# csiro-icvg/Diff3DHPE

Measured on NVIDIA B200. Metric: denoised_pose_frames_per_s, higher is better.
Workload: dtype fp16 main + block-scaled e2m1 (mxfp4) correction products (1.5 tensor-pipe units), fp32 accumulate

## Files before the change

diff3dhpe_b200/csrc/attention_tc.cu:

```cuda
#include <cstdlib>
#include "kernels.cuh"
#include "operand.cuh"
#define D3D_MBAR_SUSPEND_NS 0
#include "ptx.cuh"

namespace d3d {
namespace {

constexpr int kTcThreads = 384;
constexpr int kCtrlRegs = 40, kSoftmaxRegs = 216;
static_assert(2 * 128 * (kSoftmaxRegs - 168) <= 128 * (168 - kCtrlRegs), "setmaxnreg pool overdrawn");
constexpr int kSpatialRows = 7 * 17;
constexpr int kTile = 128 * 128;
constexpr int kSlotCols = 256;
constexpr int kOCol = 128;
constexpr float kScaleLog2e = 0.125f * 1.4426950408889634f;

constexpr int kMaxStages = 4;
template <int NSLOT>
struct TcBars {
  uint64_t full[kMaxStages];
  uint64_t stage_free[kMaxStages];
  uint64_t s_full[NSLOT];
  uint64_t p_full[NSLOT];
  uint64_t o_full[NSLOT];
  uint64_t tmem_free[NSLOT];
  uint64_t vlo_full[NSLOT];
  uint64_t staged[NSLOT];
  uint64_t stg_free[NSLOT];
  uint32_t tmem_base;
};

#ifndef D3D_ATTN_STORE_WARP
#define D3D_ATTN_STORE_WARP 1
#endif

__device__ __forceinline__ float ex2_approx(float x) {
  float y;
  asm("ex2.approx.ftz.f32 %0, %1;" : "=f"(y) : "f"(x));
  return y;
}
__device__ __forceinline__ float rcp_approx(float x) {
  float y;
  asm("rcp.approx.ftz.f32 %0, %1;" : "=f"(y) : "f"(x));
  return y;
}
__device__ __forceinline__ uint32_t pack_f16x2(float lo, float hi) {
  uint32_t r;
  asm("cvt.rn.f16x2.f32 %0, %1, %2;" : "=r"(r) : "f"(hi), "f"(lo));
  return r;
}
__device__ __forceinline__ uint64_t make_desc_mn_sw128(uint32_t smem_addr) {
  uint64_t d = 0;
  d |= static_cast<uint64_t>((smem_addr & 0x3ffffu) >> 4);
  d |= static_cast<uint64_t>(1) << 16;
  d |= static_cast<uint64_t>(1024 >> 4) << 32;
  d |= static_cast<uint64_t>(1) << 46;
  d |= static_cast<uint64_t>(2) << 61;
  return d;
}


__device__ __forceinline__ float row_sum(const ptx::f32x2 (&ls)[2]) {
  float a, b, c, d;
  ptx::unpack2(ls[0], a, b);
  ptx::unpack2(ls[1], c, d);
  return (a + b) + (c + d);
}

template <int NCH>
__device__ __forceinline__ float softmax_row(uint32_t taddr, int F, int n_chunks_rt) {
  constexpr int kMax = NCH > 0 ? NCH : 8;
  const int n = NCH > 0 ? NCH : n_chunks_rt;
  uint32_t a0[32], a1[32], b0[32], b1[32];
  float mx[4] = {-INFINITY, -INFINITY, -INFINITY, -INFINITY};
  auto full = [&](int c) { return (NCH > 0 && c < NCH - 1) || (c + 1) * 32 <= F; };
  auto max_chunk = [&](const uint32_t (&rr)[32], int c) {
    if (full(c)) {
#pragma unroll
      for (int e = 0; e < 32; ++e) mx[e & 3] = fmaxf(mx[e & 3], __uint_as_float(rr[e]));
    } else {
#pragma unroll
      for (int e = 0; e < 32; ++e)
        if (c * 32 + e < F) mx[e & 3] = fmaxf(mx[e & 3], __uint_as_float(rr[e]));
    }
  };
  ptx::tmem_ld_32x32(taddr, a0);
  if (1 < n) ptx::tmem_ld_32x32(taddr + 32, a1);
#pragma unroll
  for (int c = 0; c < kMax; c += 4) {
    if (c < n) {
      ptx::tmem_ld_wait();
      if (c + 2 < n) ptx::tmem_ld_32x32(taddr + (c + 2) * 32, b0);
      if (c + 3 < n) ptx::tmem_ld_32x32(taddr + (c + 3) * 32, b1);
      max_chunk(a0, c);
      if (c + 1 < n) max_chunk(a1, c + 1);
    }
    if (c + 2 < n) {
      ptx::tmem_ld_wait();
      if (c + 4 < n) ptx::tmem_ld_32x32(taddr + (c + 4) * 32, a0);
      if (c + 5 < n) ptx::tmem_ld_32x32(taddr + (c + 5) * 32, a1);
      max_chunk(b0, c + 2);
      if (c + 3 < n) max_chunk(b1, c + 3);
    }
  }
  ptx::tmem_ld_32x32(taddr, a0);
  if (1 < n) ptx::tmem_ld_32x32(taddr + 32, a1);
  const float nmxs = -fmaxf(fmaxf(mx[0], mx[1]), fmaxf(mx[2], mx[3])) * kScaleLog2e;
  ptx::f32x2 ls[2] = {ptx::splat2(0.f), ptx::splat2(0.f)};
  const ptx::f32x2 sc2 = ptx::splat2(kScaleLog2e), nm2 = ptx::splat2(nmxs);
  auto exp_chunk = [&](const uint32_t (&rr)[32], int c) {
    uint32_t pk[16];
    const bool whole = full(c);
#pragma unroll
    for (int e = 0; e < 16; ++e) {
      float t0, t1;
      ptx::unpack2(ptx::fma2(ptx::pack2(__uint_as_float(rr[2 * e]), __uint_as_float(rr[2 * e + 1])), sc2, nm2), t0, t1);
      const int col = c * 32 + 2 * e;
      const float e0 = (whole || col < F) ? ex2_approx(t0) : 0.f;
      const float e1 = (whole || col + 1 < F) ? ex2_approx(t1) : 0.f;
      ls[e & 1] = ptx::add2(ls[e & 1], ptx::pack2(e0, e1));
      pk[e] = pack_f16x2(e0, e1);
    }
    ptx::tmem_st_32x16(taddr + c * 16, pk);
  };
#pragma unroll
  for (int c = 0; c < kMax; c += 4) {
    if (c < n) {
      ptx::tmem_ld_wait();
      if (c + 2 < n) ptx::tmem_ld_32x32(taddr + (c + 2) * 32, b0);
      if (c + 3 < n) ptx::tmem_ld_32x32(taddr + (c + 3) * 32, b1);
      exp_chunk(a0, c);
      if (c + 1 < n) exp_chunk(a1, c + 1);
    }
    if (c + 2 < n) {
      ptx::tmem_ld_wait();
      if (c + 4 < n) ptx::tmem_ld_32x32(taddr + (c + 4) * 32, a0);
      if (c + 5 < n) ptx::tmem_ld_32x32(taddr + (c + 5) * 32, a1);
      exp_chunk(b0, c + 2);
      if (c + 3 < n) exp_chunk(b1, c + 3);
    }
  }
  ptx::tmem_st_wait();
  return rcp_approx(row_sum(ls));
}

template <int CS, int FR>
__device__ __forceinline__ float spatial_window(const uint32_t (&a)[32], const uint32_t (&b)[32], const uint32_t (&c)[32],
                                                uint32_t (&pk0)[16], uint32_t (&pk1)[16], uint32_t (&pk2)[16]) {
  constexpr int L = 17 * FR - 32 * CS;
  static_assert(L >= 0 && L + 17 <= 96, "frame window outside the loaded chunks");
  float sv[18];
#pragma unroll
  for (int k = 0; k < 17; ++k) {
    const int li = L + k;
    sv[k] = __uint_as_float(li < 32 ? a[li & 31] : li < 64 ? b[li & 31] : c[li & 31]);
  }
  sv[17] = sv[16];
  float mx = sv[0];
#pragma unroll
  for (int k = 1; k < 17; k += 2) mx = fmaxf(mx, fmaxf(sv[k], sv[k + 1]));
  const ptx::f32x2 sc2 = ptx::splat2(kScaleLog2e), nm2 = ptx::splat2(-mx * kScaleLog2e);
  float ev[18];
  ptx::f32x2 ls = ptx::splat2(0.f);
#pragma unroll
  for (int k = 0; k < 18; k += 2) {
    float t0, t1;
    ptx::unpack2(ptx::fma2(ptx::pack2(sv[k], sv[k + 1]), sc2, nm2), t0, t1);
    ev[k] = ex2_approx(t0);
    ev[k + 1] = k + 1 < 17 ? ex2_approx(t1) : 0.f;
    ls = ptx::add2(ls, ptx::pack2(ev[k], ev[k + 1]));
  }
#pragma unroll
  for (int pi = L / 2; pi <= (L + 16) / 2; ++pi) {
    const int k0 = 2 * pi - L, k1 = k0 + 1;
    const uint32_t v = pack_f16x2(k0 >= 0 && k0 < 17 ? ev[k0 < 0 ? 0 : k0] : 0.f, k1 >= 0 && k1 < 17 ? ev[k1] : 0.f);
    if (pi < 16) pk0[pi & 15] = v;
    else if (pi < 32) pk1[pi & 15] = v;
    else pk2[pi & 15] = v;
  }
  float s0, s1;
  ptx::unpack2(ls, s0, s1);
  return s0 + s1;
}

__device__ __forceinline__ float softmax_row_spatial(uint32_t taddr, int row_l, int wq) {
  const int cs = wq >> 1;
  uint32_t a[32], b[32], c[32];
  ptx::tmem_ld_32x32(taddr + cs * 32, a);
  ptx::tmem_ld_32x32(taddr + cs * 32 + 32, b);
  ptx::tmem_ld_32x32(taddr + cs * 32 + 64, c);
  uint32_t pk0[16], pk1[16], pk2[16], z[16];
#pragma unroll
  for (int e = 0; e < 16; ++e) pk0[e] = pk1[e] = pk2[e] = z[e] = 0u;
// ... 6 lines not shown
      case 1: sum = spatial_window<0, 1>(a, b, c, pk0, pk1, pk2); break;
      case 2: sum = spatial_window<0, 2>(a, b, c, pk0, pk1, pk2); break;
      default: sum = spatial_window<0, 3>(a, b, c, pk0, pk1, pk2); break;
    }
  } else {
    switch (fr) {
      case 3: sum = spatial_window<1, 3>(a, b, c, pk0, pk1, pk2); break;
      case 4: sum = spatial_window<1, 4>(a, b, c, pk0, pk1, pk2); break;
      case 5: sum = spatial_window<1, 5>(a, b, c, pk0, pk1, pk2); break;
      default: sum = spatial_window<1, 6>(a, b, c, pk0, pk1, pk2); break;
    }
  }
  __syncwarp();
  ptx::tmem_st_32x16(taddr + cs * 16, pk0);
  ptx::tmem_st_32x16(taddr + cs * 16 + 16, pk1);
  ptx::tmem_st_32x16(taddr + cs * 16 + 32, pk2);
  ptx::tmem_st_32x16(taddr + (cs == 0 ? 48 : 0), z);
  ptx::tmem_st_wait();
  return rcp_approx(sum);
}

__device__ __forceinline__ float softmax_row_packed(uint32_t taddr, int F, int G, int row_l) {
  const int jj = row_l & (G - 1);
  const uint32_t vm = (G == 4 ? 0x11111111u : 0x55555555u) << jj;
  const int nk = F * G;
  uint32_t sv[4][32];
#pragma unroll
  for (int c = 0; c < 4; ++c) ptx::tmem_ld_32x32(taddr + c * 32, sv[c]);
  ptx::tmem_ld_wait();
  float mx = -INFINITY;
#pragma unroll
  for (int c = 0; c < 4; ++c)
#pragma unroll
    for (int e = 0; e < 32; ++e)
      if (((vm >> e) & 1u) && c * 32 + e < nk) mx = fmaxf(mx, __uint_as_float(sv[c][e]));
  const ptx::f32x2 sc2 = ptx::splat2(kScaleLog2e), nm2 = ptx::splat2(-mx * kScaleLog2e);
  ptx::f32x2 ls = ptx::splat2(0.f);
#pragma unroll
  for (int c = 0; c < 4; ++c) {
    uint32_t pk[16];
#pragma unroll
    for (int e = 0; e < 16; ++e) {
      float t0, t1;
      ptx::unpack2(ptx::fma2(ptx::pack2(__uint_as_float(sv[c][2 * e]), __uint_as_float(sv[c][2 * e + 1])), sc2, nm2), t0, t1);
      const int col = c * 32 + 2 * e;
      const float e0 = (((vm >> (2 * e)) & 1u) && col < nk) ? ex2_approx(t0) : 0.f;
      const float e1 = (((vm >> (2 * e + 1)) & 1u) && col + 1 < nk) ? ex2_approx(t1) : 0.f;
      ls = ptx::add2(ls, ptx::pack2(e0, e1));
      pk[e] = pack_f16x2(e0, e1);
    }
    ptx::tmem_st_32x16(taddr + c * 16, pk);
  }
  ptx::tmem_st_wait();
  float s0, s1;
  ptx::unpack2(ls, s0, s1);
  return rcp_approx(s0 + s1);
}

template <int FMT, int NSLOT, int NCH, bool SPATIAL, bool PACKED = false>
__global__ void __launch_bounds__((4 * NSLOT + 4) * 32, 1)
attn_temporal_tc_kernel(const __grid_constant__ CUtensorMap tm_qkv, const __grid_constant__ CUtensorMap tm_hi,
                        const __grid_constant__ CUtensorMap tm_second, const __grid_constant__ CUtensorMap tm_hi_tail,
                        const __grid_constant__ CUtensorMap tm_second_tail, uint8_t* __restrict__ sf_out, int F, int J,
                        int n_units, int n_mt, int NKp, int n_stage, int pk_g = 1, int j_tok = 0) {
  static_assert(!PACKED || (!SPATIAL && NCH == 0), "the packed mode is a temporal mode with a runtime chunk count");
  static_assert(NSLOT == 2 || (NSLOT == 3 && FMT == FMT_F4C && (SPATIAL || PACKED)), "three slots: single-tile F4C modes only");
  constexpr int kSC = NSLOT == 2 ? kSlotCols : 128;
  constexpr int kOC = NSLOT == 2 ? kOCol : 64;
  constexpr int kStgSlot = NSLOT == 2 ? kTile : 8192;
  constexpr int kTmemCols = NSLOT == 2 ? 512 : 512;
  constexpr int kSmxRegs = NSLOT == 2 ? kSoftmaxRegs : 152;
  static_assert(NSLOT != 3 || 3 * 128 * (152 - 128) <= 128 * (128 - kCtrlRegs), "setmaxnreg pool overdrawn");
  extern __shared__ __align__(1024) uint8_t smem_raw[];
  uint8_t* smem = reinterpret_cast<uint8_t*>((reinterpret_cast<uintptr_t>(smem_raw) + 1023) & ~uintptr_t(1023));
  const int stage_bytes = 3 * n_mt * kTile;
  uint8_t* StgAll = smem + n_stage * stage_bytes;
  TcBars<NSLOT>* bars = reinterpret_cast<TcBars<NSLOT>*>(StgAll + NSLOT * kStgSlot);

  const int warp = threadIdx.x >> 5, lane = threadIdx.x & 31;
  constexpr int kTmaWarp = 4 * NSLOT, kMmaWarp = 4 * NSLOT + 1;
  const int n_local = blockIdx.x < n_units ? (n_units - 1 - static_cast<int>(blockIdx.x)) / static_cast<int>(gridDim.x) + 1 : 0;
  const int W = n_local * n_mt;

  if (warp == kTmaWarp && ptx::elect_one()) {
    ptx::prefetch_tensormap(&tm_qkv);
    ptx::prefetch_tensormap(&tm_hi);
    ptx::prefetch_tensormap(&tm_second);
    for (int s = 0; s < n_stage; ++s) {
      ptx::mbar_init(&bars->full[s], 1);
      ptx::mbar_init(&bars->stage_free[s], n_mt);
    }
#pragma unroll
    for (int s = 0; s < NSLOT; ++s) {
      ptx::mbar_init(&bars->s_full[s], 1);
      ptx::mbar_init(&bars->p_full[s], 128);
      ptx::mbar_init(&bars->o_full[s], 1);
      ptx::mbar_init(&bars->tmem_free[s], 128);
      ptx::mbar_init(&bars->vlo_full[s], 1);
// ... 103 lines not shown
      ptx::bulk_wait_all();
    }
  } else {
    asm volatile("setmaxnreg.inc.sync.aligned.u32 %0;" ::"n"(kSmxRegs));
    const int slot = warp >> 2;
    const int row_l = (warp & 3) * 32 + lane;
    const uint32_t taddr = tmem_base + slot * kSC + (static_cast<uint32_t>((warp & 3) * 32) << 16);
    const int n_chunks = (NKp + 31) >> 5;
    if (!SPATIAL && NCH > 0 && (n_chunks != NCH || F <= 32 * (NCH - 1))) __trap();
    if ((SPATIAL || PACKED) && (n_mt != 1 || NKp != 128)) __trap();
    const int sw = (row_l & 7) << 4;
    const bool issuer = row_l == 0;
    uint8_t* Stg = StgAll + slot * kStgSlot;
    for (int w = slot; w < W; w += NSLOT) {
      const int n = w / n_mt, m = w - n * n_mt;
      const int i = w / NSLOT, stage = n % n_stage;
      const int unit = blockIdx.x + n * gridDim.x;
      const int seq = unit >> 3, h = unit & 7;
      int b = seq / J, j = seq - b * J;
      const bool tail = SPATIAL && j == J - 1 && F % 7 != 0;
      if (SPATIAL) { j = (b * F + 7 * j) * 17; b = 0; }
      if (PACKED) j *= pk_g;
      uint8_t* Qs = smem + stage * stage_bytes;
      const uint8_t* Vs = Qs + 2 * n_mt * kTile;
      const int r = m * 128 + row_l;
      ptx::mbar_wait(&bars->s_full[slot], i & 1);
      ptx::tc_fence_after();
      if (issuer) {
        ptx::mbar_arrive_expect_tx(&bars->vlo_full[slot], kTile);
        ptx::tma_load_4d(Qs + m * kTile, &tm_qkv, &bars->vlo_full[slot], 3 * kC + h * kHd, j, m * 128, b);
      }
      const float inv = SPATIAL ? softmax_row_spatial(taddr, row_l, warp & 3)
                      : PACKED  ? softmax_row_packed(taddr, F, pk_g, row_l)
                                : softmax_row<NCH>(taddr, F, n_chunks);
      ptx::tc_fence_before();
      ptx::mbar_arrive(&bars->p_full[slot]);

      ptx::mbar_wait(&bars->vlo_full[slot], i & 1);
      uint8_t* hi_row = Qs + m * kTile + row_l * 128;
      const uint8_t* v_row = Vs + static_cast<size_t>(r) * 128;
      ptx::f32x2 nv[32];
      {
        uint4 vh[8], vl[8];
#pragma unroll
        for (int g = 0; g < 8; ++g) {
          vh[g] = *reinterpret_cast<const uint4*>(v_row + ((g << 4) ^ sw));
          vl[g] = *reinterpret_cast<const uint4*>(hi_row + ((g << 4) ^ sw));
        }
#pragma unroll
        for (int g = 0; g < 8; ++g) {
          const uint32_t vhw[4] = {vh[g].x, vh[g].y, vh[g].z, vh[g].w};
          const uint32_t vlw[4] = {vl[g].x, vl[g].y, vl[g].z, vl[g].w};
#pragma unroll
          for (int e = 0; e < 4; ++e) {
            const float2 a = __half22float2(*reinterpret_cast<const __half2*>(&vhw[e]));
            const float2 c = __half22float2(*reinterpret_cast<const __half2*>(&vlw[e]));
            float s0, s1;
            ptx::unpack2(ptx::add2(ptx::pack2(a.x, a.y), ptx::pack2(c.x, c.y)), s0, s1);
            nv[4 * g + e] = ptx::pack2(-s0, -s1);
          }
        }
      }

      ptx::mbar_wait(&bars->o_full[slot], i & 1);
      ptx::tc_fence_after();
      uint32_t o0[32], o1[32];
      ptx::tmem_ld_32x32(taddr + kOC, o0);
      ptx::tmem_ld_32x32(taddr + kOC + 32, o1);
      ptx::tmem_ld_wait();
      ptx::tc_fence_before();
      ptx::mbar_arrive(&bars->tmem_free[slot]);

      if (D3D_ATTN_STORE_WARP) {
        if (i > 0) ptx::mbar_wait(&bars->stg_free[slot], (i - 1) & 1);
      } else {
        ptx::bar_sync(1 + slot, 128);
      }
      const ptx::f32x2 inv2 = ptx::splat2(inv);
      if (FMT == FMT_F4C) {
        float ax[2] = {0.f, 0.f}, al[2] = {0.f, 0.f};
#pragma unroll
        for (int g = 0; g < 8; ++g) {
          uint32_t hw[4];
#pragma unroll
          for (int e = 0; e < 4; ++e) {
            uint32_t& ra = g < 4 ? o0[8 * g + 2 * e] : o1[8 * (g & 3) + 2 * e];
            uint32_t& rb = g < 4 ? o0[8 * g + 2 * e + 1] : o1[8 * (g & 3) + 2 * e + 1];
            float x0, x1;
            ptx::unpack2(ptx::fma2(ptx::pack2(__uint_as_float(ra), __uint_as_float(rb)), inv2, nv[4 * g + e]), x0, x1);
            const __half2 h01 = __floats2half2_rn(x0, x1);
            const float2 hf = __half22float2(h01);
            hw[e] = *reinterpret_cast<const uint32_t*>(&h01);
            ax[g >> 2] = fmaxf(ax[g >> 2], fmaxf(fabsf(x0), fabsf(x1)));
            al[g >> 2] = fmaxf(al[g >> 2], fmaxf(fabsf(x0 - hf.x), fabsf(x1 - hf.y)));
            ra = __float_as_uint(x0);
            rb = __float_as_uint(x1);
          }
          *reinterpret_cast<uint4*>(hi_row + ((g << 4) ^ sw)) = make_uint4(hw[0], hw[1], hw[2], hw[3]);
        }
        const uint32_t bp0 = op_ue8m0_of(ax[0]), bp1 = op_ue8m0_of(ax[1]), bq0 = op_ue8m0_of(al[0]), bq1 = op_ue8m0_of(al[1]);
        uint32_t pw[8], qw[8];
#pragma unroll
        for (int g = 0; g < 8; ++g) {
          const ptx::f32x2 ip = ptx::splat2(op_ue8m0_inv(g < 4 ? bp0 : bp1)), iq = ptx::splat2(op_ue8m0_inv(g < 4 ? bq0 : bq1));
          uint32_t pa = 0, qa = 0;
#pragma unroll
          for (int e = 0; e < 4; ++e) {
            const float x0 = __uint_as_float(g < 4 ? o0[8 * g + 2 * e] : o1[8 * (g & 3) + 2 * e]);
            const float x1 = __uint_as_float(g < 4 ? o0[8 * g + 2 * e + 1] : o1[8 * (g & 3) + 2 * e + 1]);
            const float2 hf = __half22float2(__floats2half2_rn(x0, x1));
            float a0, a1, l0, l1;
            ptx::unpack2(ptx::mul2(ptx::pack2(x0, x1), ip), a0, a1);
            ptx::unpack2(ptx::mul2(ptx::sub2(ptx::pack2(x0, x1), ptx::pack2(hf.x, hf.y)), iq), l0, l1);
            pa |= op_e2m1x2(a0, a1) << (8 * e);
            qa |= op_e2m1x2(l0, l1) << (8 * e);
          }
          pw[g] = pa; qw[g] = qa;
        }
        {
          uint4* stp = reinterpret_cast<uint4*>(Stg + row_l * 32);
          stp[0] = make_uint4(pw[0], pw[1], pw[2], pw[3]);
          stp[1] = make_uint4(pw[4], pw[5], pw[6], pw[7]);
          stp[256] = make_uint4(qw[0], qw[1], qw[2], qw[3]);
          stp[257] = make_uint4(qw[4], qw[5], qw[6], qw[7]);
        }
        const int pf = PACKED ? row_l / pk_g : 0, pj = PACKED ? j + (row_l & (pk_g - 1)) : 0;
        const int64_t tok = SPATIAL  ? static_cast<int64_t>(j) + row_l
// ... 462 lines not shown
}

int make_attn_tc_maps_spatial(AttnTcMaps* maps, const __half* qkv, __half* o_hi, __half* o_second, int fmt,
                              int64_t tokens, int F) {
  const int tail_rows = (F % 7) ? (F % 7) * 17 : kSpatialRows;
  if (encode_tokens_2d(&maps->o_hi_tail, o_hi, CU_TENSOR_MAP_DATA_TYPE_FLOAT16, 2, kC, tokens, tail_rows,
                       CU_TENSOR_MAP_SWIZZLE_128B))
    return -1;
  if (fmt == FMT_F8C   ? encode_tokens_2d(&maps->o_second_tail, o_second, CU_TENSOR_MAP_DATA_TYPE_UINT8, 1, 2 * kC, tokens,
                                          tail_rows, CU_TENSOR_MAP_SWIZZLE_NONE)
      : fmt == FMT_F4C ? encode_tokens_2d(&maps->o_second_tail, o_second, CU_TENSOR_MAP_DATA_TYPE_UINT8, 1, kC, tokens,
                                          tail_rows, CU_TENSOR_MAP_SWIZZLE_NONE, 32)
                       : encode_tokens_2d(&maps->o_second_tail, o_second, CU_TENSOR_MAP_DATA_TYPE_FLOAT16, 2, kC, tokens,
                                          tail_rows, CU_TENSOR_MAP_SWIZZLE_128B))
    return -1;
  if (encode_tokens_2d(&maps->qkv, const_cast<__half*>(qkv), CU_TENSOR_MAP_DATA_TYPE_FLOAT16, 2, kQkvRow, tokens, 128,
                       CU_TENSOR_MAP_SWIZZLE_128B))
    return -1;
  if (encode_tokens_2d(&maps->o_hi, o_hi, CU_TENSOR_MAP_DATA_TYPE_FLOAT16, 2, kC, tokens, kSpatialRows,
                       CU_TENSOR_MAP_SWIZZLE_128B))
    return -1;
  if (fmt == FMT_F8C)
    return encode_tokens_2d(&maps->o_second, o_second, CU_TENSOR_MAP_DATA_TYPE_UINT8, 1, 2 * kC, tokens, kSpatialRows,
                            CU_TENSOR_MAP_SWIZZLE_NONE);
  if (fmt == FMT_F4C)
    return encode_tokens_2d(&maps->o_second, o_second, CU_TENSOR_MAP_DATA_TYPE_UINT8, 1, kC, tokens, kSpatialRows,
                            CU_TENSOR_MAP_SWIZZLE_NONE, 32);
  return encode_tokens_2d(&maps->o_second, o_second, CU_TENSOR_MAP_DATA_TYPE_FLOAT16, 2, kC, tokens, kSpatialRows,
                          CU_TENSOR_MAP_SWIZZLE_128B);
}

cudaError_t configure_attention_tc() {
  cudaError_t e;
#define D3D_CFG_TC(FMT_, NCH_, SP_)                                                                                       \
  if ((e = cudaFuncSetAttribute(attn_temporal_tc_kernel<FMT_, 2, NCH_, SP_>, cudaFuncAttributeMaxDynamicSharedMemorySize, \
                                tc_smem_bytes<2>(2))) != cudaSuccess)                                                    \
    return e;
  D3D_CFG_TC(FMT_SPLIT16, 0, false) D3D_CFG_TC(FMT_F8C, 0, false) D3D_CFG_TC(FMT_SPLIT16, 3, false)
  D3D_CFG_TC(FMT_F8C, 3, false) D3D_CFG_TC(FMT_SPLIT16, 8, false) D3D_CFG_TC(FMT_F8C, 8, false)
  D3D_CFG_TC(FMT_SPLIT16, 0, true) D3D_CFG_TC(FMT_F8C, 0, true)
  D3D_CFG_TC(FMT_F4C, 0, false) D3D_CFG_TC(FMT_F4C, 3, false) D3D_CFG_TC(FMT_F4C, 8, false) D3D_CFG_TC(FMT_F4C, 0, true)
#undef D3D_CFG_TC
  if ((e = cudaFuncSetAttribute(attn_temporal_tc_kernel<FMT_F4C, 3, 0, true>, cudaFuncAttributeMaxDynamicSharedMemorySize,
                                tc_smem_bytes<3>(1))) != cudaSuccess)
    return e;
  if ((e = cudaFuncSetAttribute(attn_temporal_tc_kernel<FMT_F4C, 3, 0, false, true>, cudaFuncAttributeMaxDynamicSharedMemorySize,
                                tc_smem_bytes<3>(1))) != cudaSuccess)
    return e;
  for (auto kern : {attn_temporal_tc2_kernel<8>, attn_temporal_tc2_kernel<3>, attn_temporal_tc2_kernel<0>})
    if ((e = cudaFuncSetAttribute(kern, cudaFuncAttributeMaxDynamicSharedMemorySize, tc_smem_bytes<2>(2))) != cudaSuccess) return e;
#define D3D_CFG_PK(FMT_)                                                                                                     \
  if ((e = cudaFuncSetAttribute(attn_temporal_tc_kernel<FMT_, 2, 0, false, true>, cudaFuncAttributeMaxDynamicSharedMemorySize, \
                                tc_smem_bytes<2>(1))) != cudaSuccess)                                                        \
    return e;
  D3D_CFG_PK(FMT_SPLIT16) D3D_CFG_PK(FMT_F8C) D3D_CFG_PK(FMT_F4C)
#undef D3D_CFG_PK
  return cudaSuccess;
}

cudaError_t launch_attn_temporal_tc(const AttnTcMaps& maps, const __half* qkv, uint8_t* o_sf, int fmt, int B, int F, int J,
                                    int num_sms, cudaStream_t st, int wg2) {
  if (B <= 0) return cudaSuccess;
  if (F < 1 || F > 256) return cudaErrorInvalidValue;
  if (fmt == FMT_F4C && !o_sf) return cudaErrorInvalidValue;
  if (F <= 64) {
    const int G = packed_group(F), JG = (J + G - 1) / G;
    const int64_t units64 = static_cast<int64_t>(B) * JG * kHeads;
    if (units64 > 0x7fffffff) return cudaErrorInvalidValue;
    const int n_units = static_cast<int>(units64);
    const int grid = n_units < num_sms ? n_units : num_sms;
    const int smem = tc_smem_bytes<2>(1);
#define D3D_LAUNCH_PK(FMT_)                                                                   \
  attn_temporal_tc_kernel<FMT_, 2, 0, false, true><<<grid, kTcThreads, smem, st>>>(           \
      maps.qkv, maps.o_hi, maps.o_second, maps.o_hi, maps.o_second, o_sf, F, JG, n_units, 1, 128, tc_stages(1), G, J)
    if (fmt == FMT_F4C && three_slots())
      attn_temporal_tc_kernel<FMT_F4C, 3, 0, false, true><<<grid, 512, tc_smem_bytes<3>(1), st>>>(
          maps.qkv, maps.o_hi, maps.o_second, maps.o_hi, maps.o_second, o_sf, F, JG, n_units, 1, 128, tc_stages(1), G, J);
    else if (fmt == FMT_F4C) D3D_LAUNCH_PK(FMT_F4C);
    else if (fmt == FMT_F8C) D3D_LAUNCH_PK(FMT_F8C);
    else D3D_LAUNCH_PK(FMT_SPLIT16);
#undef D3D_LAUNCH_PK
    return cudaGetLastError();
  }
  const int n_mt = (F + 127) / 128;
  const int NKp = (F + 15) / 16 * 16;
  const int n_units = B * J * kHeads;
  const int n_chunks = (NKp + 31) / 32;
  const int nch = (n_chunks == 8 && F > 224) ? 8 : ((n_chunks == 3 && F > 64) ? 3 : 0);
  const int grid = n_units < num_sms ? n_units : num_sms;
  const int smem = tc_smem_bytes<2>(n_mt);
#define D3D_LAUNCH_TC(FMT_, NCH_)                                                                               \
  attn_temporal_tc_kernel<FMT_, 2, NCH_, false><<<grid, kTcThreads, smem, st>>>(                      \
      maps.qkv, maps.o_hi, maps.o_second, maps.o_hi, maps.o_second, o_sf, F, J, n_units, n_mt, NKp, tc_stages(n_mt))
  if (fmt == FMT_F4C && wg2) {
    if (!o_sf) return cudaErrorInvalidValue;
#define D3D_LAUNCH_TC2(NCH_)                                                       \
  attn_temporal_tc2_kernel<NCH_><<<grid, kTc2Threads, smem, st>>>(maps.qkv, maps.o_hi, maps.o_second, o_sf, F, J, n_units, \
                                                                   n_mt, NKp, tc_stages(n_mt))
    if (nch == 8) D3D_LAUNCH_TC2(8); else if (nch == 3) D3D_LAUNCH_TC2(3); else D3D_LAUNCH_TC2(0);
#undef D3D_LAUNCH_TC2
  } else if (fmt == FMT_F4C) {
    if (!o_sf) return cudaErrorInvalidValue;
    if (nch == 8) D3D_LAUNCH_TC(FMT_F4C, 8); else if (nch == 3) D3D_LAUNCH_TC(FMT_F4C, 3); else D3D_LAUNCH_TC(FMT_F4C, 0);
  } else if (fmt == FMT_F8C) {
    if (nch == 8) D3D_LAUNCH_TC(FMT_F8C, 8); else if (nch == 3) D3D_LAUNCH_TC(FMT_F8C, 3); else D3D_LAUNCH_TC(FMT_F8C, 0);
  } else {
    if (nch == 8) D3D_LAUNCH_TC(FMT_SPLIT16, 8); else if (nch == 3) D3D_LAUNCH_TC(FMT_SPLIT16, 3); else D3D_LAUNCH_TC(FMT_SPLIT16, 0);
  }
#undef D3D_LAUNCH_TC
  return cudaGetLastError();
}

cudaError_t launch_attn_spatial_tc(const AttnTcMaps& maps, uint8_t* o_sf, int fmt, int B, int F, int num_sms,
                                   cudaStream_t st) {
  if (B <= 0) return cudaSuccess;
  const int G = (F + 6) / 7;
  const int64_t units64 = static_cast<int64_t>(B) * G * kHeads;
  if (units64 > 0x7fffffff) return cudaErrorInvalidValue;
  const int n_units = static_cast<int>(units64);
  const int grid = n_units < num_sms ? n_units : num_sms;
  const int smem = tc_smem_bytes<2>(1);
  if (fmt == FMT_F4C && three_slots()) {
    if (!o_sf) return cudaErrorInvalidValue;
    attn_temporal_tc_kernel<FMT_F4C, 3, 0, true><<<grid, 512, tc_smem_bytes<3>(1), st>>>(
        maps.qkv, maps.o_hi, maps.o_second, maps.o_hi_tail, maps.o_second_tail, o_sf, F, G, n_units, 1, 128, tc_stages(1));
  } else if (fmt == FMT_F4C) {
    if (!o_sf) return cudaErrorInvalidValue;
    attn_temporal_tc_kernel<FMT_F4C, 2, 0, true><<<grid, kTcThreads, smem, st>>>(
        maps.qkv, maps.o_hi, maps.o_second, maps.o_hi_tail, maps.o_second_tail, o_sf, F, G, n_units, 1, 128, tc_stages(1));
  } else if (fmt == FMT_F8C) {
    attn_temporal_tc_kernel<FMT_F8C, 2, 0, true><<<grid, kTcThreads, smem, st>>>(
        maps.qkv, maps.o_hi, maps.o_second, maps.o_hi_tail, maps.o_second_tail, o_sf, F, G, n_units, 1, 128, tc_stages(1));
  } else {
    attn_temporal_tc_kernel<FMT_SPLIT16, 2, 0, true><<<grid, kTcThreads, smem, st>>>(
        maps.qkv, maps.o_hi, maps.o_second, maps.o_hi_tail, maps.o_second_tail, o_sf, F, G, n_units, 1, 128, tc_stages(1));
  }
  return cudaGetLastError();
}

}
```

diff3dhpe_b200/csrc/engine.cu:

```cuda
#include <cuda_fp16.h>
#include <cuda_runtime.h>

#include <algorithm>
#include <cmath>
#include <cstdio>
#include <cstdlib>
#include <cstring>
#include <map>
#include <string>
#include <vector>

#include "../../include/diff3d_b200.h"
#include "kernels.cuh"
#include "operand.cuh"

using namespace d3d;

namespace {

std::string g_create_error;

struct Lin {
  int N = 0, K = 0;
  __half* hi = nullptr;
// ... 294 lines not shown

int run_attention(d3d_handle* h, const __half* qkv, __half* o_hi, __half* o_lo, float* o_f32, int B, bool spatial,
                  int mode, cudaStream_t st) {
  const int64_t T_all = static_cast<int64_t>(B) * h->F * h->J;
  const bool tc_path = mode == D3D_ATTN_DEFAULT && qkv == h->QKV &&
                       (spatial ? (h->have_attn_sp && h->J == 17 && env_int("D3D_ATTN_TC_SPATIAL", 1))
                                : (h->have_attn_tc && env_int("D3D_ATTN_TC", 1)));
  if (h->fmt == FMT_F4C && !o_f32 && !(tc_path && attn_tc_has_f4c())) {
    if (o_hi != h->ATT.hi || o_lo != h->ATT.lo) return fail(h, -2, "attention output must be the ATT operand");
    float* scratch = reinterpret_cast<float*>(h->H.hi);
    int r = run_attention(h, qkv, nullptr, nullptr, scratch, B, spatial, mode == D3D_ATTN_DEFAULT ? D3D_ATTN_MMA_SYNC : mode, st);
    if (r) return r;
    KLP(spatial ? D3D_PROF_ATTN_SPATIAL : D3D_PROF_ATTN_TEMPORAL, st,
        launch_split(scratch, h->ATT.hi, h->ATT.lo, h->ATT.sf, T_all, kC, FMT_F4C, 0, st));
    return 0;
  }
  if (spatial) {
    if (mode == D3D_ATTN_SIMT || h->J != 17) {
      KLP(D3D_PROF_ATTN_SPATIAL, st, launch_attn_generic_simt(qkv, o_hi, o_lo, o_f32, h->fmt, B * h->F, h->J, h->J, 1, 1, st));
    } else if (tc_path && (h->fmt != FMT_F4C || attn_tc_has_f4c())) {
      if (!o_f32 && (o_hi != h->ATT.hi || o_lo != h->ATT.lo)) return fail(h, -2, "attention output must be the ATT operand");
      const int64_t T = static_cast<int64_t>(B) * h->F * h->J;
      KLP(D3D_PROF_ATTN_SPATIAL, st, launch_attn_spatial_tc(h->attn_sp, h->ATT.sf, h->fmt, B, h->F, h->num_sms, st));
      if (o_f32) KL(launch_merge(h->ATT.hi, h->ATT.lo, h->ATT.sf, o_f32, T, kC, h->fmt, st));
    } else {
      KLP(D3D_PROF_ATTN_SPATIAL, st, launch_attn_spatial(qkv, o_hi, o_lo, o_f32, h->fmt, static_cast<int64_t>(B) * h->F, h->J, st));
    }
  } else {
    if (mode == D3D_ATTN_SIMT) {
      KLP(D3D_PROF_ATTN_TEMPORAL, st, launch_attn_temporal_simt(qkv, o_hi, o_lo, o_f32, h->fmt, B, h->F, h->J, st));
    } else if (tc_path && (h->fmt != FMT_F4C || attn_tc_has_f4c())) {
      if (!o_f32 && (o_hi != h->ATT.hi || o_lo != h->ATT.lo)) return fail(h, -2, "attention output must be the ATT operand");
      KLP(D3D_PROF_ATTN_TEMPORAL, st, launch_attn_temporal_tc(h->attn_tc, qkv, h->ATT.sf, h->fmt, B, h->F, h->J, h->num_sms, st,
                                                              env_int("D3D_ATTN_WG2", 0)));
      if (o_f32) KL(launch_merge(h->ATT.hi, h->ATT.lo, h->ATT.sf, o_f32, static_cast<int64_t>(B) * h->F * h->J, kC, h->fmt, st));
    } else {
      KLP(D3D_PROF_ATTN_TEMPORAL, st, launch_attn_temporal_mma(qkv, o_hi, o_lo, o_f32, h->fmt, B, h->F, h->J, st));
    }
  }
  return 0;
}

int check_weights(d3d_handle* h) {
  static const char* per_blk[] = {"norm1.weight", "norm1.bias", "attn.qkv.weight", "attn.proj.weight", "attn.proj.bias",
                                  "norm2.weight", "norm2.bias", "mlp.fc1.weight", "mlp.fc1.bias", "mlp.fc2.weight",
                                  "mlp.fc2.bias"};
  std::vector<std::string> need = {"fusion_layer.weight", "fusion_layer.bias", "Spatial_pos_embed", "Temporal_pos_embed",
                                   "Spatial_norm.weight", "Spatial_norm.bias", "Temporal_norm.weight", "Temporal_norm.bias",
                                   "head.0.weight", "head.0.bias", "head.1.weight", "head.1.bias"};
  if (h->cfg.with_time_emb) {
    need.insert(need.end(), {"time_mlp.1.weight", "time_mlp.1.bias", "time_mlp.3.weight", "time_mlp.3.bias"});
  }
  for (int i = 0; i < h->cfg.depth; ++i)
    for (const char* kind : {"STEblocks.", "TTEblocks."}) {
      for (const char* s : per_blk) need.push_back(std::string(kind) + std::to_string(i) + "." + s);
      if (h->cfg.with_time_emb) {
        need.push_back(std::string(kind) + std::to_string(i) + ".time_mlp.1.weight");
        need.push_back(std::string(kind) + std::to_string(i) + ".time_mlp.1.bias");
      }
    }
  for (auto& n : need)
    if (!h->loaded.count(n)) return fail(h, -30, "weights not loaded: missing tensor '" + n + "'");
  for (auto& b : h->blk)
    if (b.fold_dirty) return fail(h, -30, "internal: norm2 / fc1 of a block were not folded");
  return 0;
}

// ... 908 lines not shown
```

diff3dhpe_b200/csrc/kernels.cuh:

```cuda
#pragma once
#include <cuda.h>
#include <cuda_fp16.h>
#include <cuda_runtime.h>
#include <stdint.h>

namespace d3d {

constexpr int kC = 512;
constexpr int kHeads = 8;
constexpr int kHd = 64;
constexpr int kHidden = 1024;

enum GemmEpi { EPI_F32 = 0, EPI_GELU_SPLIT = 1, EPI_QKV16 = 2, EPI_F32_LN = 3, EPI_F32_EMIT = 4, EPI_GELU_DLN = 5,
               EPI_F32_RED = 6 };

constexpr int kQkvRow = 4 * kC;

struct GemmParams {
  int M, N, K;
  const float* bias;
  const float* residual;
  float* out_f32;
  __half* out_hi;
  __half* out_lo;
// ... 67 lines not shown
cudaError_t launch_head_ddim(const float* X, LnParams post, LnParams head_ln, const float* wh ,
                             const float* bh, DdimStep s, float* y, const float* noise, float* out3,
                             float* trace_y, float* trace_x0, int trace_stride, int trace_idx, int64_t T,
                             cudaStream_t st);

cudaError_t launch_tta_merge(const float* y, const float* yf, const int32_t* perm , float scale,
                             float* out, int64_t n_frames, int J, cudaStream_t st);
cudaError_t launch_mpjpe(const float* pred, const float* gt, const uint8_t* mask, int64_t n_frames, int J,
                         double* acc, cudaStream_t st);

cudaError_t launch_pose_metrics(const float* pred, const float* gt, const int64_t* sel , int64_t n_sel, int J,
                                double* acc, double* vel_tmp, cudaStream_t st);

cudaError_t launch_window_gather(const float* seq2d, const int64_t* start, const int32_t* perm , float* x2d,
                                 float* x2d_flip , int64_t n_win, int F, int J, cudaStream_t st);
cudaError_t launch_window_scatter(const float* pred, const int64_t* start, const int32_t* first_valid, float* seq3d,
                                  int64_t n_win, int F, int J, cudaStream_t st);

cudaError_t launch_attn_spatial(const __half* qkv, __half* o_hi, __half* o_lo, float* o_f32, int fmt, int64_t n_groups,
                                int J, cudaStream_t st);
cudaError_t launch_attn_temporal_mma(const __half* qkv, __half* o_hi, __half* o_lo, float* o_f32, int fmt, int B, int F,
                                     int J, cudaStream_t st);
struct AttnTcMaps {
  CUtensorMap qkv, o_hi, o_second;
  CUtensorMap o_hi_tail, o_second_tail;
};
int make_attn_tc_maps(AttnTcMaps* maps, const __half* qkv, __half* o_hi, __half* o_second, int fmt, int F, int J,
                      int64_t max_clips);
int make_attn_tc_maps_spatial(AttnTcMaps* maps, const __half* qkv, __half* o_hi, __half* o_second, int fmt, int64_t tokens,
                              int F);
cudaError_t launch_attn_spatial_tc(const AttnTcMaps& maps, uint8_t* o_sf, int fmt, int B, int F, int num_sms, cudaStream_t st);
cudaError_t configure_attention_tc();
cudaError_t launch_attn_temporal_tc(const AttnTcMaps& maps, const __half* qkv, uint8_t* o_sf, int fmt, int B, int F, int J,
                                    int num_sms, cudaStream_t st, int wg2 = 0);
cudaError_t launch_attn_temporal_simt(const __half* qkv, __half* o_hi, __half* o_lo, float* o_f32, int fmt, int B, int F,
                                      int J, cudaStream_t st);
cudaError_t launch_attn_generic_simt(const __half* qkv, __half* o_hi, __half* o_lo, float* o_f32, int fmt, int n_seq,
                                     int N, int64_t seq_stride_tokens_outer, int inner, int64_t tok_stride,
                                     cudaStream_t st);
cudaError_t launch_pack_qkv16(const float* qkv_f32, __half* out, int64_t T, cudaStream_t st);

cudaError_t launch_t_to_f32(const int64_t* t, int R, float* out, cudaStream_t st);
cudaError_t launch_sincos(const float* t, int R, float* out, cudaStream_t st);
cudaError_t launch_small_linear(const float* in, int R, int K, const float* W, const float* b, int N, int act_in,
                                float* out, int64_t out_row_stride, cudaStream_t st);

}
```

diff3dhpe_b200/csrc/ptx.cuh:

```cuda
#pragma once
#include <cuda.h>
#include <cuda_runtime.h>
#include <stdint.h>

namespace d3d {
namespace ptx {

__device__ __forceinline__ uint32_t smem_u32(const void* p) {
  return static_cast<uint32_t>(__cvta_generic_to_shared(p));
}

__device__ __forceinline__ bool elect_one() {
  uint32_t pred = 0;
  asm volatile(
      "{\n\t"
      ".reg .pred P;\n\t"
      "elect.sync _|P, 0xffffffff;\n\t"
      "selp.u32 %0, 1, 0, P;\n\t"
      "}\n"
      : "=r"(pred));
  return pred != 0;
}

__device__ __forceinline__ void mbar_init(uint64_t* bar, uint32_t count) {
// ... 226 lines not shown
      :
      : "r"(tmem_d), "l"(desc_a), "l"(desc_b), "r"(idesc), "r"(accumulate)
      : "memory");
}
__device__ __forceinline__ void mma_f8_ss_cg2(uint32_t tmem_d, uint64_t desc_a, uint64_t desc_b, uint32_t idesc,
                                              uint32_t accumulate) {
  asm volatile(
      "{\n\t"
      ".reg .pred p;\n\t"
      "setp.ne.b32 p, %4, 0;\n\t"
      "tcgen05.mma.cta_group::2.kind::f8f6f4 [%0], %1, %2, %3, p;\n\t"
      "}\n"
      :
      : "r"(tmem_d), "l"(desc_a), "l"(desc_b), "r"(idesc), "r"(accumulate)
      : "memory");
}
__device__ __forceinline__ void mma_commit(uint64_t* bar) {
  asm volatile("tcgen05.commit.cta_group::1.mbarrier::arrive::one.shared::cluster.b64 [%0];" ::"r"(smem_u32(bar))
               : "memory");
}

__device__ __forceinline__ void tmem_ld_32x32(uint32_t taddr, uint32_t (&r)[32]) {
  asm volatile(
      "tcgen05.ld.sync.aligned.32x32b.x32.b32 "
      "{%0, %1, %2, %3, %4, %5, %6, %7, %8, %9, %10, %11, %12, %13, %14, %15, "
      "%16, %17, %18, %19, %20, %21, %22, %23, %24, %25, %26, %27, %28, %29, %30, %31}, [%32];"
      : "=r"(r[0]), "=r"(r[1]), "=r"(r[2]), "=r"(r[3]), "=r"(r[4]), "=r"(r[5]), "=r"(r[6]), "=r"(r[7]),
        "=r"(r[8]), "=r"(r[9]), "=r"(r[10]), "=r"(r[11]), "=r"(r[12]), "=r"(r[13]), "=r"(r[14]), "=r"(r[15]),
        "=r"(r[16]), "=r"(r[17]), "=r"(r[18]), "=r"(r[19]), "=r"(r[20]), "=r"(r[21]), "=r"(r[22]), "=r"(r[23]),
        "=r"(r[24]), "=r"(r[25]), "=r"(r[26]), "=r"(r[27]), "=r"(r[28]), "=r"(r[29]), "=r"(r[30]), "=r"(r[31])
      : "r"(taddr)
      : "memory");
}
__device__ __forceinline__ void tmem_ld_wait() { asm volatile("tcgen05.wait::ld.sync.aligned;" ::: "memory"); }

__device__ __forceinline__ void tma_load_4d(void* smem_dst, const CUtensorMap* m, uint64_t* bar, int32_t c0, int32_t c1,
                                            int32_t c2, int32_t c3) {
  asm volatile(
      "cp.async.bulk.tensor.4d.shared::cluster.global.mbarrier::complete_tx::bytes [%0], [%1, {%3, %4, %5, %6}], [%2];"
      :
      : "r"(smem_u32(smem_dst)), "l"(reinterpret_cast<uint64_t>(m)), "r"(smem_u32(bar)), "r"(c0), "r"(c1), "r"(c2),
        "r"(c3)
      : "memory");
}
__device__ __forceinline__ void tma_store_4d(const CUtensorMap* m, const void* smem_src, int32_t c0, int32_t c1,
                                             int32_t c2, int32_t c3) {
  asm volatile("cp.async.bulk.tensor.4d.global.shared::cta.bulk_group [%0, {%2, %3, %4, %5}], [%1];"
               :
               : "l"(reinterpret_cast<uint64_t>(m)), "r"(smem_u32(smem_src)), "r"(c0), "r"(c1), "r"(c2), "r"(c3)
               : "memory");
}
__device__ __forceinline__ void tma_prefetch_l2_2d(const CUtensorMap* m, int32_t c0, int32_t c1) {
  asm volatile("cp.async.bulk.prefetch.tensor.2d.L2.global.tile [%0, {%1, %2}];"
               :
               : "l"(reinterpret_cast<uint64_t>(m)), "r"(c0), "r"(c1)
               : "memory");
}
__device__ __forceinline__ uint4 lds128(uint32_t addr) {
  uint4 v;
  asm volatile("ld.shared.v4.b32 {%0, %1, %2, %3}, [%4];" : "=r"(v.x), "=r"(v.y), "=r"(v.z), "=r"(v.w) : "r"(addr) : "memory");
  return v;
}
__device__ __forceinline__ void sts128(uint32_t addr, uint4 v) {
  asm volatile("st.shared.v4.b32 [%0], {%1, %2, %3, %4};" ::"r"(addr), "r"(v.x), "r"(v.y), "r"(v.z), "r"(v.w) : "memory");
}
__device__ __forceinline__ void tma_reduce_add_2d(const CUtensorMap* m, uint32_t smem_src, int32_t c0, int32_t c1) {
  asm volatile("cp.reduce.async.bulk.tensor.2d.global.shared::cta.add.tile.bulk_group [%0, {%2, %3}], [%1];"
// ... 90 lines not shown
```

Baseline: 20320.

## Add opt-in one-pass temporal softmax with lazy rescale; use three-input max

Adds a one-pass softmax for the temporal attention rows. It fixes the max from the first two chunks, exponentiates every later chunk straight away, and goes back to rescale the already-stored fp16 probabilities in TMEM only when a warp's running sum passes a threshold. This removes the separate max pass over S, at the cost of a rare, warp-divergent rescale loop and some fp16 overflow risk. It also swaps pairs of fmaxf for the three-input max.f32 in the softmax, the spatial and packed windows, and the amax reductions. The one-pass path is off unless D3D_ATTN_ONEPASS is set, but the max3 change applies to the default paths.

```diff
diff --git a/diff3dhpe_b200/csrc/attention_tc.cu b/diff3dhpe_b200/csrc/attention_tc.cu
--- a/diff3dhpe_b200/csrc/attention_tc.cu
+++ b/diff3dhpe_b200/csrc/attention_tc.cu
@@ -45,6 +45,11 @@
   asm("rcp.approx.ftz.f32 %0, %1;" : "=f"(y) : "f"(x));
   return y;
 }
+__device__ __forceinline__ float fmax3(float a, float b, float c) {
+  float d;
+  asm("max.f32 %0, %1, %2, %3;" : "=f"(d) : "f"(a), "f"(b), "f"(c));
+  return d;
+}
 __device__ __forceinline__ uint32_t pack_f16x2(float lo, float hi) {
   uint32_t r;
   asm("cvt.rn.f16x2.f32 %0, %1, %2;" : "=r"(r) : "f"(hi), "f"(lo));
@@ -78,11 +83,13 @@
   auto max_chunk = [&](const uint32_t (&rr)[32], int c) {
     if (full(c)) {
 #pragma unroll
-      for (int e = 0; e < 32; ++e) mx[e & 3] = fmaxf(mx[e & 3], __uint_as_float(rr[e]));
+      for (int e = 0; e < 32; e += 2)
+        mx[(e >> 1) & 3] = fmax3(mx[(e >> 1) & 3], __uint_as_float(rr[e]), __uint_as_float(rr[e + 1]));
     } else {
 #pragma unroll
-      for (int e = 0; e < 32; ++e)
-        if (c * 32 + e < F) mx[e & 3] = fmaxf(mx[e & 3], __uint_as_float(rr[e]));
+      for (int e = 0; e < 32; e += 2)
+        mx[(e >> 1) & 3] = fmax3(mx[(e >> 1) & 3], c * 32 + e < F ? __uint_as_float(rr[e]) : -INFINITY,
+                                 c * 32 + e + 1 < F ? __uint_as_float(rr[e + 1]) : -INFINITY);
     }
   };
   ptx::tmem_ld_32x32(taddr, a0);
@@ -145,6 +152,115 @@
   return rcp_approx(row_sum(ls));
 }
 
+constexpr float kOnePassMax = 16384.f;
+template <int NCH>
+__device__ __forceinline__ float softmax_row_1p(uint32_t taddr, int F, int n_chunks_rt) {
+  constexpr int kMax = NCH > 0 ? NCH : 8;
+  const int n = NCH > 0 ? NCH : n_chunks_rt;
+  uint32_t a0[32], a1[32], b0[32], b1[32];
+  auto full = [&](int c) { return (NCH > 0 && c < NCH - 1) || (c + 1) * 32 <= F; };
+  const ptx::f32x2 sc2 = ptx::splat2(kScaleLog2e);
+  float nms = 0.f;
+  ptx::f32x2 ls[2] = {ptx::splat2(0.f), ptx::splat2(0.f)};
+  auto exp_chunk = [&](const uint32_t (&rr)[32], int c, ptx::f32x2 (&acc)[2]) {
+    const ptx::f32x2 nm2 = ptx::splat2(nms);
+    uint32_t pk[16];
+    const bool whole = full(c);
+#pragma unroll
+    for (int e = 0; e < 16; ++e) {
+      float t0, t1;
+      ptx::unpack2(ptx::fma2(ptx::pack2(__uint_as_float(rr[2 * e]), __uint_as_float(rr[2 * e + 1])), sc2, nm2), t0, t1);
+      const int col = c * 32 + 2 * e;
+      const float e0 = (whole || col < F) ? ex2_approx(t0) : 0.f;
+      const float e1 = (whole || col + 1 < F) ? ex2_approx(t1) : 0.f;
+      acc[e & 1] = ptx::add2(acc[e & 1], ptx::pack2(e0, e1));
+      pk[e] = pack_f16x2(e0, e1);
+    }
+    ptx::tmem_st_32x16(taddr + c * 16, pk);
+  };
+  auto chunk_max = [&](const uint32_t (&rr)[32], int c, float m) {
+    if (full(c)) {
+#pragma unroll
+      for (int e = 0; e < 32; e += 2) m = fmax3(m, __uint_as_float(rr[e]), __uint_as_float(rr[e + 1]));
+    } else {
+#pragma unroll
+      for (int e = 0; e < 32; e += 2)
+        m = fmax3(m, c * 32 + e < F ? __uint_as_float(rr[e]) : -INFINITY,
+                  c * 32 + e + 1 < F ? __uint_as_float(rr[e + 1]) : -INFINITY);
+    }
+    return m;
+  };
+  auto batch = [&](const uint32_t (&r0)[32], const uint32_t (&r1)[32], int c) {
+    if (c == 0) {
+      float m[4] = {-INFINITY, -INFINITY, -INFINITY, -INFINITY};
+#pragma unroll
+      for (int e = 0; e < 32; e += 2) {
+        m[(e >> 1) & 1] = fmax3(m[(e >> 1) & 1], __uint_as_float(r0[e]), __uint_as_float(r0[e + 1]));
+        m[2 + ((e >> 1) & 1)] = fmax3(m[2 + ((e >> 1) & 1)], __uint_as_float(r1[e]), __uint_as_float(r1[e + 1]));
+      }
+      nms = -fmaxf(fmax3(m[0], m[1], m[2]), m[3]) * kScaleLog2e;
+      exp_chunk(r0, 0, ls);
+      exp_chunk(r1, 1, ls);
+      return;
+    }
+    ptx::f32x2 lb[2] = {ls[0], ls[1]};
+    exp_chunk(r0, c, lb);
+    if (c + 1 < n) exp_chunk(r1, c + 1, lb);
+    float s0, s1;
+    ptx::unpack2(ptx::add2(lb[0], lb[1]), s0, s1);
+    const bool over = s0 + s1 > kOnePassMax;
+    if (!__any_sync(0xffffffffu, over)) {
+      ls[0] = lb[0];
+      ls[1] = lb[1];
+      return;
+    }
+    float d = 0.f;
+    if (over) {
+      float mb = chunk_max(r0, c, -INFINITY);
+      if (c + 1 < n) mb = chunk_max(r1, c + 1, mb);
+      d = ceilf(fmaxf(fmaf(mb, kScaleLog2e, nms), __log2f(row_sum(ls))));
+    }
+    const float f = d < 126.f ? __int_as_float((127 - static_cast<int>(d)) << 23) : 0.f;
+    ptx::tmem_st_wait();
+#pragma unroll 1
+    for (int k = 0; k < c; ++k) {
+      uint32_t p[16];
+      ptx::tmem_ld_32x16(taddr + k * 16, p);
+      ptx::tmem_ld_wait();
+#pragma unroll
+      for (int e = 0; e < 16; ++e) {
+        const float2 v = __half22float2(*reinterpret_cast<const __half2*>(&p[e]));
+        p[e] = pack_f16x2(v.x * f, v.y * f);
+      }
+      ptx::tmem_st_32x16(taddr + k * 16, p);
+    }
+    nms -= d;
+    ls[0] = ptx::mul2(ls[0], ptx::splat2(f));
+    ls[1] = ptx::mul2(ls[1], ptx::splat2(f));
+    exp_chunk(r0, c, ls);
+    if (c + 1 < n) exp_chunk(r1, c + 1, ls);
+  };
+  ptx::tmem_ld_32x32(taddr, a0);
+  ptx::tmem_ld_32x32(taddr + 32, a1);
+#pragma unroll
+  for (int c = 0; c < kMax; c += 4) {
+    if (c < n) {
+      ptx::tmem_ld_wait();
+      if (c + 2 < n) ptx::tmem_ld_32x32(taddr + (c + 2) * 32, b0);
+      if (c + 3 < n) ptx::tmem_ld_32x32(taddr + (c + 3) * 32, b1);
+      batch(a0, a1, c);
+    }
+    if (c + 2 < n) {
+      ptx::tmem_ld_wait();
+      if (c + 4 < n) ptx::tmem_ld_32x32(taddr + (c + 4) * 32, a0);
+      if (c + 5 < n) ptx::tmem_ld_32x32(taddr + (c + 5) * 32, a1);
+      batch(b0, b1, c + 2);
+    }
+  }
+  ptx::tmem_st_wait();
+  return rcp_approx(row_sum(ls));
+}
+
 template <int CS, int FR>
 __device__ __forceinline__ float spatial_window(const uint32_t (&a)[32], const uint32_t (&b)[32], const uint32_t (&c)[32],
                                                 uint32_t (&pk0)[16], uint32_t (&pk1)[16], uint32_t (&pk2)[16]) {
@@ -159,7 +275,7 @@
   sv[17] = sv[16];
   float mx = sv[0];
 #pragma unroll
-  for (int k = 1; k < 17; k += 2) mx = fmaxf(mx, fmaxf(sv[k], sv[k + 1]));
+  for (int k = 1; k < 17; k += 2) mx = fmax3(mx, sv[k], sv[k + 1]);
   const ptx::f32x2 sc2 = ptx::splat2(kScaleLog2e), nm2 = ptx::splat2(-mx * kScaleLog2e);
   float ev[18];
   ptx::f32x2 ls = ptx::splat2(0.f);
@@ -232,8 +348,9 @@
 #pragma unroll
   for (int c = 0; c < 4; ++c)
 #pragma unroll
-    for (int e = 0; e < 32; ++e)
-      if (((vm >> e) & 1u) && c * 32 + e < nk) mx = fmaxf(mx, __uint_as_float(sv[c][e]));
+    for (int e = 0; e < 32; e += 2)
+      mx = fmax3(mx, (((vm >> e) & 1u) && c * 32 + e < nk) ? __uint_as_float(sv[c][e]) : -INFINITY,
+                 (((vm >> (e + 1)) & 1u) && c * 32 + e + 1 < nk) ? __uint_as_float(sv[c][e + 1]) : -INFINITY);
   const ptx::f32x2 sc2 = ptx::splat2(kScaleLog2e), nm2 = ptx::splat2(-mx * kScaleLog2e);
   ptx::f32x2 ls = ptx::splat2(0.f);
 #pragma unroll
@@ -257,13 +374,14 @@
   return rcp_approx(s0 + s1);
 }
 
-template <int FMT, int NSLOT, int NCH, bool SPATIAL, bool PACKED = false>
+template <int FMT, int NSLOT, int NCH, bool SPATIAL, bool PACKED = false, bool ONEPASS = false>
 __global__ void __launch_bounds__((4 * NSLOT + 4) * 32, 1)
 attn_temporal_tc_kernel(const __grid_constant__ CUtensorMap tm_qkv, const __grid_constant__ CUtensorMap tm_hi,
                         const __grid_constant__ CUtensorMap tm_second, const __grid_constant__ CUtensorMap tm_hi_tail,
                         const __grid_constant__ CUtensorMap tm_second_tail, uint8_t* __restrict__ sf_out, int F, int J,
                         int n_units, int n_mt, int NKp, int n_stage, int pk_g = 1, int j_tok = 0) {
   static_assert(!PACKED || (!SPATIAL && NCH == 0), "the packed mode is a temporal mode with a runtime chunk count");
+  static_assert(!ONEPASS || (!SPATIAL && !PACKED), "the one-pass softmax is the temporal mode's (F > 64)");
   static_assert(NSLOT == 2 || (NSLOT == 3 && FMT == FMT_F4C && (SPATIAL || PACKED)), "three slots: single-tile F4C modes only");
   constexpr int kSC = NSLOT == 2 ? kSlotCols : 128;
   constexpr int kOC = NSLOT == 2 ? kOCol : 64;
@@ -433,6 +551,7 @@
       }
       const float inv = SPATIAL ? softmax_row_spatial(taddr, row_l, warp & 3)
                       : PACKED  ? softmax_row_packed(taddr, F, pk_g, row_l)
+                      : ONEPASS ? softmax_row_1p<NCH>(taddr, F, n_chunks)
                                 : softmax_row<NCH>(taddr, F, n_chunks);
       ptx::tc_fence_before();
       ptx::mbar_arrive(&bars->p_full[slot]);
@@ -492,8 +611,8 @@
             const __half2 h01 = __floats2half2_rn(x0, x1);
             const float2 hf = __half22float2(h01);
             hw[e] = *reinterpret_cast<const uint32_t*>(&h01);
-            ax[g >> 2] = fmaxf(ax[g >> 2], fmaxf(fabsf(x0), fabsf(x1)));
-            al[g >> 2] = fmaxf(al[g >> 2], fmaxf(fabsf(x0 - hf.x), fabsf(x1 - hf.y)));
+            ax[g >> 2] = fmax3(ax[g >> 2], fabsf(x0), fabsf(x1));
+            al[g >> 2] = fmax3(al[g >> 2], fabsf(x0 - hf.x), fabsf(x1 - hf.y));
             ra = __float_as_uint(x0);
             rb = __float_as_uint(x1);
           }
@@ -1022,14 +1141,16 @@
 
 cudaError_t configure_attention_tc() {
   cudaError_t e;
-#define D3D_CFG_TC(FMT_, NCH_, SP_)                                                                                       \
-  if ((e = cudaFuncSetAttribute(attn_temporal_tc_kernel<FMT_, 2, NCH_, SP_>, cudaFuncAttributeMaxDynamicSharedMemorySize, \
-                                tc_smem_bytes<2>(2))) != cudaSuccess)                                                    \
+#define D3D_CFG_TC(FMT_, NCH_, SP_, OP_)                                                                                  \
+  if ((e = cudaFuncSetAttribute(attn_temporal_tc_kernel<FMT_, 2, NCH_, SP_, false, OP_>,                                 \
+                                cudaFuncAttributeMaxDynamicSharedMemorySize, tc_smem_bytes<2>(2))) != cudaSuccess)      \
     return e;
-  D3D_CFG_TC(FMT_SPLIT16, 0, false) D3D_CFG_TC(FMT_F8C, 0, false) D3D_CFG_TC(FMT_SPLIT16, 3, false)
-  D3D_CFG_TC(FMT_F8C, 3, false) D3D_CFG_TC(FMT_SPLIT16, 8, false) D3D_CFG_TC(FMT_F8C, 8, false)
-  D3D_CFG_TC(FMT_SPLIT16, 0, true) D3D_CFG_TC(FMT_F8C, 0, true)
-  D3D_CFG_TC(FMT_F4C, 0, false) D3D_CFG_TC(FMT_F4C, 3, false) D3D_CFG_TC(FMT_F4C, 8, false) D3D_CFG_TC(FMT_F4C, 0, true)
+  D3D_CFG_TC(FMT_SPLIT16, 0, true, false) D3D_CFG_TC(FMT_F8C, 0, true, false) D3D_CFG_TC(FMT_F4C, 0, true, false)
+#define D3D_CFG_TEMPORAL(FMT_)                                                                                           \
+  D3D_CFG_TC(FMT_, 0, false, false) D3D_CFG_TC(FMT_, 3, false, false) D3D_CFG_TC(FMT_, 8, false, false)                \
+  D3D_CFG_TC(FMT_, 0, false, true) D3D_CFG_TC(FMT_, 3, false, true) D3D_CFG_TC(FMT_, 8, false, true)
+  D3D_CFG_TEMPORAL(FMT_SPLIT16) D3D_CFG_TEMPORAL(FMT_F8C) D3D_CFG_TEMPORAL(FMT_F4C)
+#undef D3D_CFG_TEMPORAL
 #undef D3D_CFG_TC
   if ((e = cudaFuncSetAttribute(attn_temporal_tc_kernel<FMT_F4C, 3, 0, true>, cudaFuncAttributeMaxDynamicSharedMemorySize,
                                 tc_smem_bytes<3>(1))) != cudaSuccess)
@@ -1049,7 +1170,7 @@
 }
 
 cudaError_t launch_attn_temporal_tc(const AttnTcMaps& maps, const __half* qkv, uint8_t* o_sf, int fmt, int B, int F, int J,
-                                    int num_sms, cudaStream_t st, int wg2) {
+                                    int num_sms, cudaStream_t st, int wg2, int onepass) {
   if (B <= 0) return cudaSuccess;
   if (F < 1 || F > 256) return cudaErrorInvalidValue;
   if (fmt == FMT_F4C && !o_sf) return cudaErrorInvalidValue;
@@ -1079,9 +1200,14 @@
   const int nch = (n_chunks == 8 && F > 224) ? 8 : ((n_chunks == 3 && F > 64) ? 3 : 0);
   const int grid = n_units < num_sms ? n_units : num_sms;
   const int smem = tc_smem_bytes<2>(n_mt);
-#define D3D_LAUNCH_TC(FMT_, NCH_)                                                                               \
-  attn_temporal_tc_kernel<FMT_, 2, NCH_, false><<<grid, kTcThreads, smem, st>>>(                      \
+#define D3D_LAUNCH_TC1(FMT_, NCH_, OP_)                                                                  \
+  attn_temporal_tc_kernel<FMT_, 2, NCH_, false, false, OP_><<<grid, kTcThreads, smem, st>>>(             \
       maps.qkv, maps.o_hi, maps.o_second, maps.o_hi, maps.o_second, o_sf, F, J, n_units, n_mt, NKp, tc_stages(n_mt))
+#define D3D_LAUNCH_TC(FMT_, NCH_)             \
+  do {                                        \
+    if (onepass) D3D_LAUNCH_TC1(FMT_, NCH_, true); \
+    else D3D_LAUNCH_TC1(FMT_, NCH_, false);   \
+  } while (0)
   if (fmt == FMT_F4C && wg2) {
     if (!o_sf) return cudaErrorInvalidValue;
 #define D3D_LAUNCH_TC2(NCH_)                                                       \
@@ -1098,6 +1224,7 @@
     if (nch == 8) D3D_LAUNCH_TC(FMT_SPLIT16, 8); else if (nch == 3) D3D_LAUNCH_TC(FMT_SPLIT16, 3); else D3D_LAUNCH_TC(FMT_SPLIT16, 0);
   }
 #undef D3D_LAUNCH_TC
+#undef D3D_LAUNCH_TC1
   return cudaGetLastError();
 }
 
diff --git a/diff3dhpe_b200/csrc/engine.cu b/diff3dhpe_b200/csrc/engine.cu
--- a/diff3dhpe_b200/csrc/engine.cu
+++ b/diff3dhpe_b200/csrc/engine.cu
@@ -350,7 +350,7 @@
     } else if (tc_path && (h->fmt != FMT_F4C || attn_tc_has_f4c())) {
       if (!o_f32 && (o_hi != h->ATT.hi || o_lo != h->ATT.lo)) return fail(h, -2, "attention output must be the ATT operand");
       KLP(D3D_PROF_ATTN_TEMPORAL, st, launch_attn_temporal_tc(h->attn_tc, qkv, h->ATT.sf, h->fmt, B, h->F, h->J, h->num_sms, st,
-                                                              env_int("D3D_ATTN_WG2", 0)));
+                                                              env_int("D3D_ATTN_WG2", 0), env_int("D3D_ATTN_ONEPASS", 0)));
       if (o_f32) KL(launch_merge(h->ATT.hi, h->ATT.lo, h->ATT.sf, o_f32, static_cast<int64_t>(B) * h->F * h->J, kC, h->fmt, st));
     } else {
       KLP(D3D_PROF_ATTN_TEMPORAL, st, launch_attn_temporal_mma(qkv, o_hi, o_lo, o_f32, h->fmt, B, h->F, h->J, st));
diff --git a/diff3dhpe_b200/csrc/kernels.cuh b/diff3dhpe_b200/csrc/kernels.cuh
--- a/diff3dhpe_b200/csrc/kernels.cuh
+++ b/diff3dhpe_b200/csrc/kernels.cuh
@@ -123,7 +123,7 @@
 cudaError_t launch_attn_spatial_tc(const AttnTcMaps& maps, uint8_t* o_sf, int fmt, int B, int F, int num_sms, cudaStream_t st);
 cudaError_t configure_attention_tc();
 cudaError_t launch_attn_temporal_tc(const AttnTcMaps& maps, const __half* qkv, uint8_t* o_sf, int fmt, int B, int F, int J,
-                                    int num_sms, cudaStream_t st, int wg2 = 0);
+                                    int num_sms, cudaStream_t st, int wg2 = 0, int onepass = 0);
 cudaError_t launch_attn_temporal_simt(const __half* qkv, __half* o_hi, __half* o_lo, float* o_f32, int fmt, int B, int F,
                                       int J, cudaStream_t st);
 cudaError_t launch_attn_generic_simt(const __half* qkv, __half* o_hi, __half* o_lo, float* o_f32, int fmt, int n_seq,
diff --git a/diff3dhpe_b200/csrc/ptx.cuh b/diff3dhpe_b200/csrc/ptx.cuh
--- a/diff3dhpe_b200/csrc/ptx.cuh
+++ b/diff3dhpe_b200/csrc/ptx.cuh
@@ -282,7 +282,16 @@
       : "r"(taddr)
       : "memory");
 }
-__device__ __forceinline__ void tmem_ld_wait() { asm volatile("tcgen05.wait::ld.sync.aligned;" ::: "memory"); }
+__device__ __forceinline__ void tmem_ld_32x16(uint32_t taddr, uint32_t (&r)[16]) {
+  asm volatile(
+      "tcgen05.ld.sync.aligned.32x32b.x16.b32 "
+      "{%0, %1, %2, %3, %4, %5, %6, %7, %8, %9, %10, %11, %12, %13, %14, %15}, [%16];"
+      : "=r"(r[0]), "=r"(r[1]), "=r"(r[2]), "=r"(r[3]), "=r"(r[4]), "=r"(r[5]), "=r"(r[6]), "=r"(r[7]),
+        "=r"(r[8]), "=r"(r[9]), "=r"(r[10]), "=r"(r[11]), "=r"(r[12]), "=r"(r[13]), "=r"(r[14]), "=r"(r[15])
+      : "r"(taddr)
+      : "memory");
+}
+__device__ __forceinline__ void tmem_ld_wait(){ asm volatile("tcgen05.wait::ld.sync.aligned;" ::: "memory"); }
 
 __device__ __forceinline__ void tma_load_4d(void* smem_dst, const CUtensorMap* m, uint64_t* bar, int32_t c0, int32_t c1,
                                             int32_t c2, int32_t c3) {
```

Measured after the change: 20310 (median of 6 runs). About the same (-0.0%).
